# OpenVectorAI/CoFHE

Hardware: AMD Instinct MI355X
Metric: ciphertext-ops/sec + HBM GB/s (% roofline), 128x128 matadd (higher is better)
Workload: dtype u32; 1 GPU; ciphertext_matadd 128x128 per GPU (C2), security 128, k 128, |Delta| = 2088 bits, valid ciphertexts of random plaintexts; elements_per_gpu=16384, parallelism=row-shard x1, collective=none

## Files before the change

__graft_entry__.py:

```python
import json
import os
import subprocess
import sys

ROOT = os.path.dirname(os.path.abspath(__file__))
CSRC = os.path.join(ROOT, "cofhe_amd", "csrc")
LIB = os.path.join(ROOT, "cofhe_amd", "libcofhe_hip.so")
HIP_SOURCES = ["cofhe_hip.hip", "abi.hip", "kernels.hpp", "wire.hip", "shard.hip", "wide.hip", "ctx.hpp", "lane.hpp", "mp.hpp", "qf.hpp",
               "form_io.hpp", "layout.hpp", "wide.hpp", "qfw.hpp", "comb.hip", "comb.hpp", "affine.hip", "affine.hpp", "wg_ctx.hpp",
               "matmul_left.hip", "plain_mm.hpp", "conv.hip", "conv.hpp", "pow_dot.hip", "pow_dot.hpp", "poly_shift.hpp",
               "divide.hip", "plain_div.hpp", "lut.hip", "lut.hpp", "wire.hpp"]
HIP_OBJECTS = [("part0", "cofhe_hip.hip", ["-DCOFHE_PART=0"]), ("part1", "cofhe_hip.hip", ["-DCOFHE_PART=1"]),
               ("part2", "cofhe_hip.hip", ["-DCOFHE_PART=2"]), ("abi", "abi.hip", []), ("wire", "wire.hip", []), ("shard", "shard.hip", []),
               ("wide", "wide.hip", []), ("comb", "comb.hip", []), ("affine", "affine.hip", []),
               ("matmul_left", "matmul_left.hip", []), ("conv", "conv.hip", []), ("pow_dot", "pow_dot.hip", []),
               ("divide", "divide.hip", []), ("lut", "lut.hip", [])]


def _stale(target, deps):
    if not os.path.exists(target):
        return True
    t = os.path.getmtime(target)
    return any(os.path.getmtime(d) > t for d in deps)


def build_library(src_dir, obj_dir, lib, extra_flags=()) -> None:
    hipcc = os.environ.get("HIPCC", "/opt/rocm/bin/hipcc")
    flags = ["--offload-arch=gfx950", "-O2", "-std=c++17", "-fPIC", "-Wno-unused-value"] + list(extra_flags)
    os.makedirs(obj_dir, exist_ok=True)
    jobs = []
    for name, src, extra in HIP_OBJECTS:
        obj = os.path.join(obj_dir, name + ".o")
        jobs.append((obj, subprocess.Popen([hipcc] + flags + extra + ["-c", os.path.join(src_dir, src), "-o", obj], cwd=ROOT)))
    for obj, pr in jobs:
        if pr.wait() != 0:
            raise subprocess.CalledProcessError(pr.returncode, "hipcc -c -> " + obj)
    subprocess.check_call([hipcc, "--offload-arch=gfx950", "-shared", "-fPIC", "-o", lib] + [o for o, _ in jobs] + ["-ldl"], cwd=ROOT)


def build() -> None:
    deps = [os.path.join(CSRC, f) for f in HIP_SOURCES] + [os.path.join(ROOT, "include", "cofhe_hip.h")]
    if _stale(LIB, deps):
        build_library(CSRC, os.path.join(CSRC, "obj"), LIB)
    odir = os.path.join(ROOT, "oracle")
    if _stale(os.path.join(odir, "libcofhe_oracle.so"),
              [os.path.join(odir, "cofhe_oracle.hpp"), os.path.join(odir, "cofhe_oracle_c.cpp")]):
        subprocess.check_call(["make", "-C", odir])
    hdir = os.path.join(ROOT, "cofhe_amd", "host")
    exe = os.path.join(hdir, "local_bench")
    if _stale(exe, [os.path.join(hdir, f) for f in ("local_bench.cpp", "hip_cryptosystem.hpp", "smpc_local.hpp", "tensor.hpp")] + [LIB]):
        subprocess.check_call(["g++", "-std=c++17", "-O2", "-I/opt/conda/include", "-o", exe,
                               os.path.join(hdir, "local_bench.cpp"), "-L" + os.path.join(ROOT, "cofhe_amd"),
                               "-lcofhe_hip", "-l:libgmp.so.10", "-Wl,-rpath,$ORIGIN/.."], cwd=hdir)
    gdir = os.path.join(ROOT, "tests", "gpu_kernels")
    gso = os.path.join(gdir, "liblehmer_gpu.so")
    if _stale(gso, [os.path.join(gdir, "lehmer_gpu.hip"), os.path.join(CSRC, "mp.hpp"), os.path.join(CSRC, "lane.hpp")]):
        subprocess.check_call([os.environ.get("HIPCC", "/opt/rocm/bin/hipcc"), "--offload-arch=gfx950", "-O2", "-std=c++17", "-fPIC", "-shared",
                               "-Wno-unused-value", "-o", gso, os.path.join(gdir, "lehmer_gpu.hip")], cwd=ROOT)
    psrc = os.path.join(gdir, "prims_gpu.hip")
    pso = os.path.join(gdir, "libprims_gpu.so")
    pdeps = ["lane.hpp", "mp.hpp", "qf.hpp", "layout.hpp", "form_io.hpp", "wide.hpp", "qfw.hpp", "wg_ctx.hpp"]
    if os.path.exists(psrc) and _stale(pso, [psrc] + [os.path.join(CSRC, f) for f in pdeps]):
        subprocess.check_call([os.environ.get("HIPCC", "/opt/rocm/bin/hipcc"), "--offload-arch=gfx950", "-O2", "-std=c++17", "-fPIC", "-shared",
                               "-Wno-unused-value", "-o", pso, psrc], cwd=ROOT)
    lsrc = os.path.join(gdir, "lowmul_gpu.hip")
    lso = os.path.join(gdir, "liblowmul_gpu.so")
    if os.path.exists(lsrc) and _stale(lso, [lsrc] + [os.path.join(CSRC, f) for f in ("lane.hpp", "mp.hpp", "qf.hpp")]):
        subprocess.check_call([os.environ.get("HIPCC", "/opt/rocm/bin/hipcc"), "--offload-arch=gfx950", "-O2", "-std=c++17", "-fPIC", "-shared",
                               "-Wno-unused-value", "-o", lso, lsrc], cwd=ROOT)
    osrc = os.path.join(gdir, "onep_gpu.hip")
    oso = os.path.join(gdir, "libonep_gpu.so")
    if os.path.exists(osrc) and _stale(oso, [osrc] + [os.path.join(CSRC, f) for f in ("lane.hpp", "mp.hpp", "qf.hpp")]):
        subprocess.check_call([os.environ.get("HIPCC", "/opt/rocm/bin/hipcc"), "--offload-arch=gfx950", "-O2", "-std=c++17", "-fPIC", "-shared",
                               "-Wno-unused-value", "-o", oso, osrc], cwd=ROOT)
    sys.path.insert(0, ROOT)
    import cofhe_amd
    cofhe_amd.load_library()


def smoke() -> None:
    sys.path.insert(0, ROOT)
    sys.path.insert(0, os.path.join(ROOT, "tests"))
    from cofhe_amd import Engine
    import oracle_lib as O

    def hx(s):
        return -int(s[1:], 16) if s.startswith("-") else int(s, 16)

    g = os.path.join(ROOT, "tests", "golden")
    prm = json.load(open(os.path.join(g, "params_s128_k128.json")))
    vec = json.load(open(os.path.join(g, "vectors_s128_k128.json")))
    d = hx(prm["delta"])
    eng = Engine(d, device=0)
    v = vec["add_valid"]
    t1, t2 = bytes.fromhex(v["ct1"]), bytes.fromhex(v["ct2"])
    out = eng.add_ciphertext_tensors(t1, t2)
    assert out == bytes.fromhex(v["out"]), "HIP add != golden"
    assert out == O.add(d, t1, t2), "HIP add != oracle"
    v = vec["scal_2d"]
    out = eng.scal_ciphertext_tensors(bytes.fromhex(v["s"]), bytes.fromhex(v["cts"]), bytes.fromhex(v["zero"]))
    assert out == bytes.fromhex(v["out"]), "HIP scal matmul != golden"
    print("smoke ok: add_ciphertext_tensors and scal_ciphertext_tensors match golden vectors and oracle")


if __name__ == "__main__":
    build()
    if len(sys.argv) > 1 and sys.argv[1] == "smoke":
        smoke()
```

cofhe_amd/csrc/lane.hpp:

```cpp
#pragma once
#include <stdint.h>

#if defined(COFHE_HOSTSIM)
#include <atomic>
#include <cmath>
#include <cstdio>
#include <cstdlib>
#include <thread>
#define CF_DEV inline
#define CF_DEV_COLD inline
#define CF_UNROLL _Pragma("GCC unroll 16")
#define CF_NOUNROLL
#else
#include <hip/hip_runtime.h>
#define CF_DEV __device__ __forceinline__
#ifdef COFHE_COLD_CALLS
#define CF_DEV_COLD __device__ __attribute__((noinline, cold))
#else
#define CF_DEV_COLD __device__ __forceinline__
#endif
#define CF_UNROLL _Pragma("unroll")
#define CF_NOUNROLL _Pragma("nounroll")
#endif

// ... 45 lines not shown
                }
            }
        }
    }
};

struct GroupShared {
    alignas(64) uint32_t xchg[G];
    alignas(64) uint32_t own_scratch[SCRATCH_WORDS];
    uint32_t *scratch = own_scratch;
    SpinBarrier bar;
};

struct WgShared {
    SpinBarrier bar;
    SpinBarrier wave_bar;
    uint32_t vote[64];
    int wave_threads = 0;
};

struct Ctx {
    int gl;
    GroupShared *gs;
    int sense = 0;
    WgShared *wg = nullptr;
    int wg_sense = 0, wave_sense = 0;
    int tid = 0;
    uint32_t *wg_mail = nullptr, *wg_scr0 = nullptr;
    int gi = 0, wave = 0, rank = -1;
    uint32_t *scratch() const { return gs->scratch; }
};

CF_DEV void group_sync(Ctx &c) { c.gs->bar.wait(c.sense); }

CF_DEV uint32_t shfl(Ctx &c, uint32_t v, int src) {
    c.gs->xchg[c.gl] = v;
    c.gs->bar.wait(c.sense);
    uint32_t r = c.gs->xchg[src & (G - 1)];
    c.gs->bar.wait(c.sense);
    return r;
}
CF_DEV uint32_t shfl_up1(Ctx &c, uint32_t v, uint32_t fill) {
    uint32_t r = shfl(c, v, (c.gl + G - 1) & (G - 1));
    return c.gl == 0 ? fill : r;
}
CF_DEV uint32_t shfl_down1(Ctx &c, uint32_t v, uint32_t fill) {
    uint32_t r = shfl(c, v, (c.gl + 1) & (G - 1));
    return c.gl == G - 1 ? fill : r;
}
CF_DEV uint32_t shfl_xor1(Ctx &c, uint32_t v) { return shfl(c, v, c.gl ^ 1); }
CF_DEV uint32_t shfl_xor2(Ctx &c, uint32_t v) { return shfl(c, v, c.gl ^ 2); }
CF_DEV uint32_t shfl_mirror(Ctx &c, uint32_t v) { return shfl(c, v, (G - 1) - c.gl); }
CF_DEV uint32_t shfl_down4(Ctx &c, uint32_t v) { return shfl(c, v, c.gl + G / 2); }
CF_DEV uint32_t bcast_first(Ctx &c, uint32_t v) { return shfl(c, v, 0); }
CF_DEV uint32_t bcast_last(Ctx &c, uint32_t v) { return shfl(c, v, G - 1); }
CF_DEV uint32_t ballot8(Ctx &c, bool p) {
    uint32_t m = 0;
    c.gs->xchg[c.gl] = p ? 1u : 0u;
    c.gs->bar.wait(c.sense);
    for (int i = 0; i < G; i++) m |= c.gs->xchg[i] << i;
    c.gs->bar.wait(c.sense);
    return m;
}

#else

struct Ctx {
    int gl;
    int base4;
    uint32_t *scr;
    uint32_t *wg_mail = nullptr;
    uint32_t *wg_scr0 = nullptr;
    int gi = 0, wave = 0;
    int rank = 0;
    uint32_t *status = nullptr;
#ifdef COFHE_WG_TIMING
    unsigned long long t_wait = 0, t_apply = 0, n_rounds = 0, t_serve = 0;
#endif
    __device__ uint32_t *scratch() const { return scr; }
};
#define CF_ST_EUCLID_CAP 1u
#define CF_ST_REDUCE_CAP 2u
#define CF_ST_DIV_CAP 4u
#define CF_ST_BAD_FORM 8u
#define CF_ST_SCHEDULE_CAP 16u
#if !defined(COFHE_HOSTSIM)
#define CF_STATUS(c, bits) do { if ((c).status && (c).gl == 0) atomicOr((c).status, (bits)); } while (0)
#endif
#ifdef COFHE_WG_TIMING
#define CF_PHASE(id) do { if (threadIdx.x == 0) g_wg_phase[blockIdx.x * 16 + (id)] = wall_clock64(); } while (0)
#define CF_PHASE_VAL(id, v) do { if (threadIdx.x == 0) g_wg_phase[blockIdx.x * 16 + (id)] = (v); } while (0)
#define CF_FLAG(bits) do { if (c.gl == 0) atomicOr(&g_wg_flags[blockIdx.x], (bits)); } while (0)
#else
#define CF_PHASE(id) do { } while (0)
#define CF_PHASE_VAL(id, v) do { } while (0)
#define CF_FLAG(bits) do { } while (0)
#endif

CF_DEV void group_sync(Ctx &) {
    __builtin_amdgcn_fence(__ATOMIC_RELEASE, "wavefront");
    __builtin_amdgcn_wave_barrier();
    __builtin_amdgcn_fence(__ATOMIC_ACQUIRE, "wavefront");
}

CF_DEV uint32_t shfl(Ctx &c, uint32_t v, int src) {
    return (uint32_t)__builtin_amdgcn_ds_bpermute(c.base4 + ((src & (G - 1)) << 2), (int)v);
}
CF_DEV uint32_t shfl_up1(Ctx &c, uint32_t v, uint32_t fill) {
    uint32_t r = (uint32_t)__builtin_amdgcn_update_dpp((int)fill, (int)v, 0x111, 0xF, 0xF, false);
    return c.gl == 0 ? fill : r;
}
CF_DEV uint32_t shfl_down1(Ctx &c, uint32_t v, uint32_t fill) {
    uint32_t r = (uint32_t)__builtin_amdgcn_update_dpp((int)fill, (int)v, 0x101, 0xF, 0xF, false);
    return c.gl == G - 1 ? fill : r;
}
CF_DEV uint32_t shfl_xor1(Ctx &, uint32_t v) {
    return (uint32_t)__builtin_amdgcn_mov_dpp((int)v, 0xB1, 0xF, 0xF, true);
}
CF_DEV uint32_t shfl_xor2(Ctx &, uint32_t v) {
    return (uint32_t)__builtin_amdgcn_mov_dpp((int)v, 0x4E, 0xF, 0xF, true);
}
CF_DEV uint32_t shfl_mirror(Ctx &, uint32_t v) {
    return (uint32_t)__builtin_amdgcn_mov_dpp((int)v, 0x141, 0xF, 0xF, true);
}
CF_DEV uint32_t shfl_down4(Ctx &, uint32_t v) {
    return (uint32_t)__builtin_amdgcn_update_dpp((int)v, (int)v, 0x104, 0xF, 0xF, false);
}
CF_DEV uint32_t bcast_first(Ctx &, uint32_t v) {
    const int q = __builtin_amdgcn_mov_dpp((int)v, 0x00, 0xF, 0xF, true);
    return (uint32_t)__builtin_amdgcn_update_dpp(q, q, 0x141, 0xF, 0xA, false);
}
CF_DEV uint32_t bcast_last(Ctx &, uint32_t v) {
    const int q = __builtin_amdgcn_mov_dpp((int)v, 0xFF, 0xF, 0xF, true);
    return (uint32_t)__builtin_amdgcn_update_dpp(q, q, 0x141, 0xF, 0x5, false);
}
CF_DEV uint32_t ballot8(Ctx &c, bool p) {
    uint64_t m = __builtin_amdgcn_ballot_w64(p);
    return (uint32_t)(m >> (c.base4 >> 2)) & ((1u << G) - 1u);
}

#endif

CF_DEV uint32_t bcast(Ctx &c, uint32_t v, int src) { return shfl(c, v, src); }

CF_DEV bool any_lane(Ctx &c, bool p) {
#if defined(COFHE_HOSTSIM)
    return ballot8(c, p) != 0;
#else
    (void)c;
    return __builtin_amdgcn_ballot_w64(p) != 0;
#endif
}

CF_DEV uint32_t group_max(Ctx &c, uint32_t v) {
    uint32_t o;
    o = shfl_xor1(c, v); v = o > v ? o : v;
    o = shfl_xor2(c, v); v = o > v ? o : v;
    o = shfl_mirror(c, v); v = o > v ? o : v;
    return v;
}

CF_DEV int clz32(uint32_t x) { return x ? __builtin_clz(x) : 32; }

}
```

cofhe_amd/csrc/mp.hpp:

```cpp
#pragma once
#include "lane.hpp"

namespace cofhe {

#if defined(COFHE_HOSTSIM)
struct SimStats { long batches, batch_steps, divsteps, muls, divrems, resolves, bits_gained; };
inline SimStats g_stats;
#define CF_STAT(x) do { if (c.gl == 0) { x; } } while (0)
#else
#define CF_STAT(x) do { } while (0)
#endif

CF_DEV uint32_t opaque(uint32_t v) {
#if defined(COFHE_HOSTSIM)
    asm volatile("" : "+r"(v));
#else
    asm volatile("" : "+v"(v));
#endif
    return v;
}

template <int P>
struct Mp {
    uint32_t v[P][CH];
// ... 480 lines not shown
            const int k = first ? k0 + t : k1 + t - n0;
            const uint32_t *px = s + (first ? 0 : 2 * HL) + ((first ? c.gl : oc1) - k) * CH;
            const uint32_t *py = s + (first ? HL : 3 * HL) + k * CH;
            uint32_t xc[CH], yc[CH];
            CF_UNROLL for (int j = 0; j < CH; j++) {
                xc[j] = px[j];
                yc[j] = py[j];
            }
            chunk_mac(w, xc, yc);
            const bool last_of_first = (t + 1 == n0);
            CF_UNROLL for (int i = 0; i < W; i++) w0[i] = last_of_first ? w[i] : w0[i];
        }
        uint32_t bw = 0;
        CF_UNROLL for (int i = 0; i < W; i++) {
            const uint64_t d = (uint64_t)w[i] - w0[i] - bw;
            w1[i] = (uint32_t)d;
            bw = (uint32_t)(d >> 63);
        }
    }
    group_sync(c);
    uint32_t *s1 = s + G * (CH + 1);
    CF_UNROLL for (int i = 0; i < CH + 1; i++) s[c.gl * (CH + 1) + i] = w0[CH + i];
    CF_UNROLL for (int i = 0; i < W; i++) s1[oc1 * W + i] = w1[i];
    group_sync(c);
    Mp<2> r;
    uint32_t hi[2];
    {
        uint32_t cy = 0, cz = 0;
        CF_UNROLL for (int j = 0; j < CH; j++) {
            const uint32_t up = (c.gl >= 1) ? s[(c.gl >= 1 ? c.gl - 1 : 0) * (CH + 1) + j] : 0u;
            const uint32_t ov = (j == 0 && c.gl >= 2) ? s[(c.gl >= 2 ? c.gl - 2 : 0) * (CH + 1) + CH] : 0u;
            const uint64_t t = (uint64_t)w0[j] + up + ov + cy;
            r.v[0][j] = (uint32_t)t;
            cy = (uint32_t)(t >> 32);
            const uint32_t up1 = (c.gl >= 1) ? s1[(c.gl >= 1 ? c.gl - 1 : 0) * W + CH + j] : 0u;
            const uint32_t ov1 = (j == 0 && c.gl >= 2) ? s1[(c.gl >= 2 ? c.gl - 2 : 0) * W + 2 * CH] : 0u;
            const uint64_t u = (uint64_t)s1[c.gl * W + j] + up1 + ov1 + cz;
            r.v[1][j] = (uint32_t)u;
            cz = (uint32_t)(u >> 32);
        }
        hi[0] = cy;
        hi[1] = cz;
    }
    group_sync(c);
    (void)mp_resolve_sparse(c, r, hi);
    MpPair pp;
    CF_UNROLL for (int j = 0; j < CH; j++) {
        pp.p0.v[0][j] = r.v[0][j];
        pp.p1.v[0][j] = r.v[1][j];
    }
    return pp;
}

CF_DEV Mp<1> mp_sqr_low(Ctx &c, const Mp<1> &x) {
    static_assert(PLIMBS + G <= SCRATCH_WORDS && G * (CH + 1) <= SCRATCH_WORDS, "scratch too small");
    CF_STAT(g_stats.muls += 1);
    uint32_t *s = c.scratch();
    CF_UNROLL for (int j = 0; j < CH; j++) s[c.gl * CH + j] = x.v[0][j];
    s[PLIMBS + c.gl] = 0u;
    group_sync(c);
    const int kx = (mp_bitlen(c, x) + CH * 32 - 1) / (CH * 32);
    uint32_t w[2 * CH + 1];
    CF_UNROLL for (int i = 0; i < 2 * CH + 1; i++) w[i] = 0;
    CF_NOUNROLL for (int k = 0; k < kx; k++) {
        const uint32_t *px = s + ((c.gl - k) & (G - 1)) * CH;
        const uint32_t *py = (k <= c.gl) ? s + k * CH : s + PLIMBS;
        uint32_t xc[CH], yc[CH];
        CF_UNROLL for (int j = 0; j < CH; j++) {
            xc[j] = px[j];
            yc[j] = py[j];
        }
        chunk_mac(w, xc, yc);
    }
    group_sync(c);
    CF_UNROLL for (int i = 0; i < CH + 1; i++) s[c.gl * (CH + 1) + i] = w[CH + i];
    group_sync(c);
    Mp<1> r;
    uint32_t hi[1];
    {
        uint32_t cy = 0;
        CF_UNROLL for (int j = 0; j < CH; j++) {
            const uint32_t up = (c.gl >= 1) ? s[(c.gl >= 1 ? c.gl - 1 : 0) * (CH + 1) + j] : 0u;
            const uint32_t ov = (j == 0 && c.gl >= 2) ? s[(c.gl >= 2 ? c.gl - 2 : 0) * (CH + 1) + CH] : 0u;
            const uint64_t t = (uint64_t)w[j] + up + ov + cy;
            r.v[0][j] = (uint32_t)t;
            cy = (uint32_t)(t >> 32);
        }
        hi[0] = cy;
    }
    group_sync(c);
    (void)mp_resolve_sparse(c, r, hi);
    return r;
}

CF_DEV uint64_t div64_lower(uint64_t n, uint64_t d) {
    double q = (double)(n & ~0x7FFull) / (double)d;
    uint64_t t = (uint64_t)q;
    return t > 0 ? t - 1 : 0;
}

template <int PN, int PD>
CF_DEV uint32_t mp_quot_digit(Ctx &c, const Mp<PN> &num, int nb, const Mp<PD> &den, int db, int &sh) {
    int npos = nb > 64 ? nb - 64 : 0;
    int dpos = db > 32 ? db - 32 : 0;
    uint64_t nt = mp_bits64(c, num, npos);
    uint64_t dt = (uint64_t)mp_bits32(c, den, dpos) + (dpos > 0 ? 1u : 0u);
    int e = npos - dpos;
    uint64_t t;
    if (CF_UNLIKELY(dt == 0)) {
        CF_STATUS(c, CF_ST_DIV_CAP);
        sh = 0;
        return 1;
    }
    if (dpos == 0 && npos == 0) {
        t = nt / dt;
    } else {
        t = div64_lower(nt, dt);
    }
    if (e < 0) {
        t = (-e >= 64) ? 0 : (t >> (-e));
        e = 0;
    }
    int extra = 33 - __builtin_clzll(t | 1);
    if (extra > 0) {
        t >>= extra;
// ... 286 lines not shown
        WordDiv d = worddiv_make(mp_get_limb(c, den, 0));
        quot = num;
        uint32_t r = mp_divrem_word(c, quot, d);
        mp_set_word(c, num, r);
        return;
    }
    if constexpr (PD == 1) {
        mp_divrem_norm(c, num, den, db, quot);
        return;
    }
    if (db < 64) {
        mp_divrem_cons(c, num, den, quot);
        return;
    }
    mp_zero(quot);
    const int nb = mp_bitlen(c, num);
    if (nb < db) return;
    uint32_t *s = c.scratch();
    CF_UNROLL for (int p = 0; p < PD; p++)
        CF_UNROLL for (int j = 0; j < CH; j++) s[p * PLIMBS + c.gl * CH + j] = den.v[p][j];
    group_sync(c);
    const uint64_t d64 = mp_bits64(c, den, db - 64);
    const double rd = 1.0 / (double)d64;
    for (int jq = (nb - db) / 32; jq >= 0; jq--) {
        CF_STAT(g_stats.divsteps++);
        const int pos = db - 64 + 32 * jq;
        const uint64_t hi64 = mp_bits64(c, num, pos + 32);
        const uint32_t lo32 = mp_bits32(c, num, pos);
        double x = ((double)hi64 * 4294967296.0 + (double)lo32) * rd;
        x += x * 1.7763568394002505e-15;
        uint64_t qd = (uint64_t)x;
        if (qd > 0xFFFFFFFFull) qd = 0xFFFFFFFFull;
        if (qd != 0) {
            Mp<PN> ds;
            CF_UNROLL for (int p = 0; p < PN; p++)
                CF_UNROLL for (int j = 0; j < CH; j++) {
                    int i = p * PLIMBS + c.gl * CH + j - jq;
                    bool ok = i >= 0 && i < PD * PLIMBS;
                    ds.v[p][j] = ok ? s[ok ? i : 0] : 0u;
                }
            mp_lincomb_sub(c, num, 1u, num, (uint32_t)qd, ds);
            for (int fix = 0; fix < 4 && ballot8(c, c.gl == G - 1 && (num.v[PN - 1][CH - 1] >> 31)) != 0; fix++) {
                (void)mp_add(c, num, num, ds);
                qd--;
            }
        }
        CF_UNROLL for (int p = 0; p < PN; p++)
            CF_UNROLL for (int j = 0; j < CH; j++)
                quot.v[p][j] = (p * PLIMBS + c.gl * CH + j == jq) ? (uint32_t)qd : quot.v[p][j];
    }
    group_sync(c);
}

template <int PN, int PQ>
CF_DEV void mp_divexact(Ctx &c, const Mp<PN> &num, const Mp<1> &den, Mp<PQ> &quot, int nq) {
    static_assert((PN + PQ) * PLIMBS <= SCRATCH_WORDS, "scratch too small");
    mp_zero(quot);
    if (nq <= 0) return;
    if (nq > PQ * PLIMBS) nq = PQ * PLIMBS;
    const uint32_t d0raw = bcast_first(c, den.v[0][0]);
    if (CF_UNLIKELY(d0raw == 0)) {
        Mp<PN> rem = num, q;
        mp_divrem(c, rem, den, q);
        quot = mp_resize<PQ>(q);
        return;
    }
    const int tz = __builtin_ctz(d0raw);
    const Mp<1> D = mp_shr_small(c, den, tz);
    const Mp<PN> Nn = mp_shr_small(c, num, tz);
    const uint32_t d0 = d0raw >> tz | (tz ? bcast_first(c, den.v[0][1]) << (32 - tz) : 0u);
    uint32_t dinv = d0;
    CF_UNROLL for (int i = 0; i < 4; i++) dinv *= 2u - d0 * dinv;
    uint32_t *sn = c.scratch(), *sq = sn + PN * PLIMBS;
    CF_UNROLL for (int p = 0; p < PN; p++)
        CF_UNROLL for (int j = 0; j < CH; j++) sn[p * PLIMBS + c.gl * CH + j] = Nn.v[p][j];
    CF_UNROLL for (int p = 0; p < PQ; p++)
        CF_UNROLL for (int j = 0; j < CH; j++) sq[p * PLIMBS + c.gl * CH + j] = 0u;
    group_sync(c);
    Mp<1> S;
    CF_UNROLL for (int j = 0; j < CH; j++) S.v[0][j] = Nn.v[0][j];
    int64_t adj = 0;
    auto high = [&](int k) -> uint32_t { return (PLIMBS + k < PN * PLIMBS) ? sn[(PLIMBS + k < PN * PLIMBS) ? PLIMBS + k : 0] : 0u; };
    const uint64_t d64 = ((uint64_t)bcast_first(c, D.v[0][1]) << 32) | d0;
    uint64_t dinv64 = dinv;
    dinv64 *= 2ull - d64 * dinv64;
    int i = 0;
    for (; i + 1 < nq; i += 2) {
        CF_STAT(g_stats.divsteps += 2);
        const uint64_t s01 = ((uint64_t)bcast_first(c, S.v[0][1]) << 32) | bcast_first(c, S.v[0][0]);
        const uint64_t q = s01 * dinv64;
        const uint32_t q0 = (uint32_t)q, q1 = (uint32_t)(q >> 32);
        uint32_t r1[CH];
        const uint32_t hi1 = lincomb_plane<true>(r1, 1u, S.v[0], q0, D.v[0], c.gl == 0 ? q0 : 0u);
        const int64_t v1 = (int64_t)high(i) + adj + (int64_t)bcast_last(c, hi1) - (int64_t)q0;
        const int64_t adj1 = v1 >> 32;
        const uint32_t inc = shfl_up1(c, hi1, 0u);
        const uint32_t r0 = r1[0] + inc;
        const uint32_t bit = r0 < inc ? 1u : 0u;
        uint32_t s2[CH];
        s2[CH - 1] = shfl_down1(c, r0, (uint32_t)v1);
        CF_UNROLL for (int j = 0; j + 1 < CH; j++) s2[j] = r1[j + 1];
        Mp<1> T;
        uint32_t hi2[1];
        hi2[0] = lincomb_plane<true>(T.v[0], 1u, s2, q1, D.v[0], c.gl == 0 ? q1 : bit);
        const uint32_t cw = mp_resolve(c, T, hi2);
        const int64_t v2 = (int64_t)high(i + 1) + adj1 + (int64_t)cw - (int64_t)q1;
        adj = v2 >> 32;
        const uint32_t up = shfl_down1(c, T.v[0][0], (uint32_t)v2);
        CF_UNROLL for (int j = 0; j + 1 < CH; j++) S.v[0][j] = T.v[0][j + 1];
        S.v[0][CH - 1] = up;
        if (c.gl == 0) {
            sq[i] = q0;
            sq[i + 1] = q1;
        }
    }
    for (; i < nq; i++) {
        CF_STAT(g_stats.divsteps++);
        const uint32_t q = bcast_first(c, S.v[0][0]) * dinv;
        Mp<1> T;
        const uint32_t cw = mp_lincomb_sub_carry(c, T, 1u, S, q, D);
        const int64_t v = (int64_t)high(i) + adj + (int64_t)cw - (int64_t)q;
        adj = v >> 32;
        const uint32_t up = shfl_down1(c, T.v[0][0], (uint32_t)v);
        CF_UNROLL for (int j = 0; j + 1 < CH; j++) S.v[0][j] = T.v[0][j + 1];
        S.v[0][CH - 1] = up;
        if (c.gl == 0) sq[i] = q;
    }
    group_sync(c);
    CF_UNROLL for (int p = 0; p < PQ; p++)
        CF_UNROLL for (int j = 0; j < CH; j++) quot.v[p][j] = sq[p * PLIMBS + c.gl * CH + j];
    group_sync(c);
}

template <int P>
CF_DEV void smp_add(Ctx &c, SMp<P> &r, const SMp<P> &x, const SMp<P> &y) {
    if (x.neg == y.neg) {
        (void)mp_add(c, r.m, x.m, y.m);
        r.neg = x.neg;
    } else {
        int cm = mp_cmp(c, x.m, y.m);
        if (cm >= 0) {
            Mp<P> t;
            mp_sub(c, t, x.m, y.m);
            r.m = t;
            r.neg = cm == 0 ? 0 : x.neg;
        } else {
            Mp<P> t;
            mp_sub(c, t, y.m, x.m);
            r.m = t;
            r.neg = y.neg;
        }
    }
}
template <int P>
CF_DEV void smp_sub(Ctx &c, SMp<P> &r, const SMp<P> &x, const SMp<P> &y) {
    SMp<P> ny = y;
    ny.neg ^= 1;
    smp_add(c, r, x, ny);
}
template <int P, int Q>
CF_DEV SMp<P + Q> smp_mul(Ctx &c, const SMp<P> &x, const SMp<Q> &y) {
    SMp<P + Q> r;
    r.m = mp_mul(c, x.m, y.m);
    r.neg = x.neg ^ y.neg;
    return r;
}

CF_DEV void mp_bits64_pair(Ctx &c, const Mp<1> &x, const Mp<1> &y, int pos, uint64_t &xh, uint64_t &yh) {
    uint32_t *s = c.scratch();
    CF_UNROLL for (int j = 0; j < CH; j++) {
        s[c.gl * CH + j] = x.v[0][j];
        s[PLIMBS + c.gl * CH + j] = y.v[0][j];
    }
    s[2 * PLIMBS + c.gl] = 0u;
    group_sync(c);
    const int i0 = pos >> 5, o = pos & 31;
    const int i1 = i0 + 1 < PLIMBS ? i0 + 1 : 2 * PLIMBS, i2 = i0 + 2 < PLIMBS ? i0 + 2 : 2 * PLIMBS;
    const uint32_t x0 = s[i0], x1 = s[i1 < PLIMBS ? i1 : 2 * PLIMBS], x2 = s[i2 < PLIMBS ? i2 : 2 * PLIMBS];
    const uint32_t y0 = s[PLIMBS + i0], y1 = s[i1 < PLIMBS ? PLIMBS + i1 : 2 * PLIMBS],
                   y2 = s[i2 < PLIMBS ? PLIMBS + i2 : 2 * PLIMBS];
    group_sync(c);
    const uint64_t xl = ((uint64_t)x1 << 32) | x0, yl = ((uint64_t)y1 << 32) | y0;
    xh = o ? ((xl >> o) | ((uint64_t)x2 << (64 - o))) : xl;
    yh = o ? ((yl >> o) | ((uint64_t)y2 << (64 - o))) : yl;
// ... 408 lines not shown
```

cofhe_amd/csrc/qf.hpp:

```cpp
#pragma once
#include "mp.hpp"

namespace cofhe {

struct QForm {
    Mp<1> a;
    Mp<1> bm;
    int bneg;
    Mp<2> c;
};

template <int P>
CF_DEV void qf_reduce(Ctx &c, Mp<P> &a, SMp<P> &b, Mp<P> &cc) {
    for (int guard = 0;; guard++) {
        if (CF_UNLIKELY(guard > 4 * P * PLIMBS * 32)) {
            CF_STATUS(c, CF_ST_REDUCE_CAP);
            return;
        }
        int cm = mp_cmp(c, b.m, a);
        if (cm > 0 || (cm == 0 && b.neg)) {
            Mp<P> two_a;
            (void)mp_add(c, two_a, a, a);
            if (mp_cmp(c, b.m, two_a) < 0) {
                Mp<P> t;
// ... 64 lines not shown
}
CF_DEV bool m12_low_half_serves(int nb, uint32_t v1_limb0) {
    if (v1_limb0 == 0) return false;
    return nb + 1 + __builtin_ctz(v1_limb0) <= LOW2_BITS;
}
CF_DEV SMp<1> m12_low_quot(Ctx &c, const Mp<1> &pp, bool sub, int neg0, const Mp<1> &v1, int nb) {
    if (nb < 0) {
        SMp<1> z;
        mp_zero(z.m);
        z.neg = 0;
        return z;
    }
    const bool low = c.gl < LOW2_CHUNKS;
    const uint32_t flip = sub ? 0xFFFFFFFFu : 0u;
    Mp<1> n;
    uint32_t hi[1];
    {
        uint32_t cy = (sub && c.gl == 0) ? 1u : 0u;
        CF_UNROLL for (int j = 0; j < CH; j++) {
            const uint64_t t = (uint64_t)pp.v[0][j] + (shfl_down4(c, pp.v[0][j]) ^ flip) + cy;
            n.v[0][j] = (uint32_t)t;
            cy = (uint32_t)(t >> 32);
        }
        hi[0] = low ? cy : 0u;
    }
    CF_UNROLL for (int j = 0; j < CH; j++) n.v[0][j] = low ? n.v[0][j] : 0u;
    (void)mp_resolve(c, n, hi);
    CF_UNROLL for (int j = 0; j < CH; j++) n.v[0][j] = low ? n.v[0][j] : 0u;
    Mp<1> q;
    mp_divexact(c, n, v1, q, (nb + 32) >> 5);
    const int topl = nb >> 5;
    const uint32_t topmask = (2u << (nb & 31)) - 1u;
    uint32_t sbit = 0;
    CF_UNROLL for (int j = 0; j < CH; j++) sbit |= (c.gl * CH + j == topl) ? (q.v[0][j] >> (nb & 31)) & 1u : 0u;
    const bool neg = ballot8(c, sbit != 0) != 0;
    const uint32_t inv = neg ? 0xFFFFFFFFu : 0u;
    SMp<1> r;
    {
        uint32_t cy = (neg && c.gl == 0) ? 1u : 0u;
        CF_UNROLL for (int j = 0; j < CH; j++) {
            const int l = c.gl * CH + j;
            const uint32_t mask = l < topl ? 0xFFFFFFFFu : (l == topl ? topmask : 0u);
            const uint64_t t = (uint64_t)((q.v[0][j] ^ inv) & mask) + cy;
            r.m.v[0][j] = (uint32_t)t;
            cy = (uint32_t)(t >> 32);
        }
        hi[0] = cy;
    }
    (void)mp_resolve(c, r.m, hi);
    r.neg = neg0 ^ (neg ? 1 : 0);
    return r;
}

#ifdef COFHE_M12_FULL
constexpr bool M12_LOW_HALF = false;
#else
constexpr bool M12_LOW_HALF = true;
#endif

CF_DEV bool nucomp_m12(Ctx &c, SMp<1> &M1, SMp<2> &M2, const Mp<1> &R, const SMp<1> &C, const Mp<1> &v1,
                       const Mp<1> &v2, const SMp<1> &m, const SMp<1> &s, const Mp<2> &c2d, int lv1, int lv2, bool try_low) {
    if (M12_LOW_HALF && try_low) {
        const int bR = mp_bitlen(c, R), bC = mp_bitlen(c, C.m);
        const int nb1 = m12_bound(lv2, bR, mp_bitlen(c, m.m), bC, lv1);
        const int nb2 = m12_bound(mp_bitlen(c, s.m), bR, mp_bitlen(c, c2d), bC, lv1);
        const uint32_t v1w = bcast_first(c, v1.v[0][0]);
        const bool ok = m12_low_half_serves(nb1, v1w) && m12_low_half_serves(nb2, v1w);
        if (CF_LIKELY(!any_lane(c, !ok))) {
            const Mp<1> pa = mp_mul_low2(c, v2, R, m.m, C.m);
            M1 = m12_low_quot(c, pa, m.neg == C.neg, 0, v1, nb1);
            const Mp<1> pb = mp_mul_low2(c, s.m, R, mp_resize<1>(c2d), C.m);
            const SMp<1> q2 = m12_low_quot(c, pb, s.neg != C.neg, s.neg, v1, nb2);
            M2.m = mp_resize<2>(q2.m);
            M2.neg = q2.neg;
            return true;
        }
    }
    SMp<1> Rs{R, 0};
    SMp<1> v2s{v2, 0};
    SMp<2> t1 = smp_mul(c, v2s, Rs);
    SMp<2> t2 = smp_mul(c, m, C);
    SMp<2> n1;
    smp_sub(c, n1, t1, t2);
    M1 = sdiv_exact<1>(c, n1, v1);
    SMp<2> t3 = smp_mul(c, s, Rs);
    SMp<2> c2s{c2d, 0};
    SMp<3> t4w = smp_mul(c, c2s, C);
    SMp<2> t4{mp_resize<2>(t4w.m), t4w.neg};
    SMp<2> n2;
    smp_add(c, n2, t3, t4);
    M2 = sdiv_exact<2>(c, n2, v1);
    return false;
}

CF_DEV SMp<2> nucomp_dot(Ctx &c, const Mp<1> &R, const SMp<1> &C, const SMp<1> &M1, const SMp<2> &M2, bool m2_one_plane) {
    SMp<1> Rs{R, 0};
    SMp<2> p1 = smp_mul(c, Rs, M1);
    SMp<2> p2;
    if (M12_LOW_HALF && CF_LIKELY(m2_one_plane)) {
        const SMp<1> M2l{mp_resize<1>(M2.m), M2.neg};
        p2 = smp_mul(c, C, M2l);
    } else {
        SMp<3> p2w = smp_mul(c, C, M2);
        p2.m = mp_resize<2>(p2w.m);
        p2.neg = p2w.neg;
    }
    SMp<2> r;
    smp_add(c, r, p1, p2);
    return r;
}

#ifdef COFHE_DOT_FULL
constexpr bool DOT_ONE_PLANE = false;
#else
constexpr bool DOT_ONE_PLANE = true;
#endif
constexpr int DOT1_PRODUCT_BITS = PLIMBS * 32 - 3;
CF_DEV bool dot_one_plane_serves(int bR, int bC, int bM1, int bM2) {
    return bR <= LOW2_BITS && bC <= LOW2_BITS && bM1 <= LOW2_BITS && bM2 <= LOW2_BITS && bR + bM1 <= DOT1_PRODUCT_BITS &&
           bC + bM2 <= DOT1_PRODUCT_BITS;
}
// ... 335 lines not shown
                x2.m = x2p.m; x2.neg = x2p.neg ^ s.neg;
                SMp<1> sabs{s.m, 0};
                SMp<2> t = smp_mul(c, x2p, sabs);
                SMp<2> d1w{mp_resize<2>(d1), 0};
                SMp<2> t2;
                smp_sub(c, t2, t, d1w);
                y2 = sdiv_exact<1>(c, t2, d);
            }
        }
        if (mp_is_word(c, d1, 1)) {
            v1 = f1.a; v2 = f2.a; c2d = f2.c;
        } else {
            Mp<1> qq;
            v1 = f1.a; mp_divrem(c, v1, d1, qq); v1 = qq;
            v2 = f2.a; mp_divrem(c, v2, d1, qq); v2 = qq;
            Mp<3> cw = mp_mul(c, f2.c, d1);
            c2d = mp_resize<2>(cw);
        }
        const SMp<1> r0s{r, 1};
        SMp<2> num = smp_mul(c, y2, r0s);
        if (x2w != 0) {
            SMp<2> u, df;
            (void)mp_lincomb_add(c, u.m, x2w, f2.c, 0u, f2.c);
            u.neg = x2.neg;
            smp_sub(c, df, num, u);
            num = df;
        } else if (!mp_is_zero(c, x2.m)) {
            SMp<2> c2s{f2.c, 0};
            SMp<1> c2r{smod(c, c2s, v1), 0};
            SMp<2> w3 = smp_mul(c, x2, c2r), df;
            smp_sub(c, df, num, w3);
            num = df;
        }
        r = smod(c, num, v1);
    }

    CF_PHASE(3);
    const int lv1 = mp_bitlen(c, v1), lv2 = mp_bitlen(c, v2);
    int stop = (lv1 - lv2 + half_dbits) / 2;
    Euclid<1> pe;
    pe.x = v1; pe.y = r;
    mp_zero(pe.ux); mp_set_word(c, pe.uy, 1);
    pe.sx = -1; pe.sy = 1;
    qf_euclid<WG>(c, pe, stop);
    CF_PHASE(4);
#ifdef COFHE_WG_TIMING
    CF_PHASE_VAL(10, c.t_wait); CF_PHASE_VAL(11, c.t_apply); CF_PHASE_VAL(13, c.n_rounds); CF_PHASE_VAL(15, c.t_serve);
    c.t_wait = 0; c.t_apply = 0; c.n_rounds = 0; c.t_serve = 0;
#endif
    const SMp<1> C0{pe.ux, pe.sx < 0}, C1{pe.uy, pe.sy < 0};

    SMp<1> M1;
    SMp<2> M2;
    const bool m2_one_plane = nucomp_m12(c, M1, M2, pe.y, C1, v1, v2, m, s, c2d, lv1, lv2, true);
    SMp<2> an, bn;
    const bool ab_one_plane = nucomp_ab<ONE_PLANE>(c, an, bn, pe.y, C1, pe.x, C0, M1, M2, b1, m2_one_plane);
    SMp<2> cn;
    CF_PHASE(5);
    if (CF_LIKELY(ab_one_plane || (mp_high_planes_zero(c, an.m, 1) && mp_high_planes_zero(c, bn.m, 1)))) {
        (void)nucomp_c<ONE_PLANE>(c, cn.m, mp_resize<1>(an.m), mp_resize<1>(bn.m), dd);
        cn.neg = 0;
    } else {
        SMp<1> M1p;
        SMp<2> M2p;
        (void)nucomp_m12(c, M1p, M2p, pe.x, C0, v1, v2, m, s, c2d, lv1, lv2, false);
        cn = nucomp_dot(c, pe.x, C0, M1p, M2p, false);
    }

    CF_PHASE(6);
    if (CF_LIKELY(mp_bitlen(c, an.m) < PLIMBS * 32 - 8 && mp_bitlen(c, bn.m) < PLIMBS * 32 - 8 &&
                  mp_bitlen(c, cn.m) < PLIMBS * 32 - 8)) {
        Mp<1> a1 = mp_resize<1>(an.m), c1 = mp_resize<1>(cn.m);
        SMp<1> b1r{mp_resize<1>(bn.m), bn.neg};
        qf_reduce<1>(c, a1, b1r, c1);
        out.a = a1;
        out.bm = b1r.m;
        out.bneg = b1r.neg;
        out.c = mp_resize<2>(c1);
    } else {
        qf_reduce<2>(c, an.m, bn, cn.m);
        out.a = mp_resize<1>(an.m);
        out.bm = mp_resize<1>(bn.m);
        out.bneg = bn.neg;
        out.c = cn.m;
    }
    CF_PHASE(7);
}

CF_DEV void qf_inverse(Ctx &c, QForm &f) {
    if (mp_is_zero(c, f.bm)) return;
    if (mp_cmp(c, f.bm, f.a) == 0) return;
    if (mp_cmp(c, mp_resize<2>(f.a), f.c) == 0) return;
    f.bneg ^= 1;
}

constexpr uint32_t QF_BAD_SIGN_WORD = 1u << 0, QF_BAD_POSITIVE = 1u << 1, QF_BAD_B_LE_A = 1u << 2, QF_BAD_A_LE_C = 1u << 3,
                   QF_BAD_EDGE_SIGN = 1u << 4, QF_BAD_ZERO_SIGN = 1u << 5, QF_BAD_CARRY = 1u << 6, QF_BAD_LOW_BITS = 1u << 7,
                   QF_BAD_EQUATION = 1u << 8, QF_BAD_PRIMITIVE = 1u << 9;

CF_DEV uint32_t qf_form_faults(Ctx &c, const QForm &f, const uint32_t *absdelta) {
    uint32_t bad = 0;
    if (!(f.bneg == 0 || f.bneg == 1)) bad |= QF_BAD_SIGN_WORD;
    if (mp_is_zero(c, f.a)) bad |= QF_BAD_POSITIVE;
    if (mp_is_zero(c, f.c)) bad |= QF_BAD_POSITIVE;
    const Mp<2> aw = mp_resize<2>(f.a);
    const int ba = mp_cmp(c, f.bm, f.a), ac = mp_cmp(c, aw, f.c);
    if (ba > 0) bad |= QF_BAD_B_LE_A;
// ... 92 lines not shown
```

Before: 51.78 million ciphertext-ops/s.

## Pair the two M1/M2 exact divisions across lane halves and halve squaring work

Computes the two low-half NUCOMP quotients (M1, M2) together, one per half of the 8-lane group, through new paired resolve, shift and 2-limb-per-step exact-division routines. This replaces two sequential divisions. It also rewrites mp_sqr_low to compute each cross product once, double the sum, then add the diagonal terms. mp_divexact now skips high-word bookkeeping when the numerator is a single plane. The matadd benchmark may not exercise the NUCOMP path, and the new lane-half code depends on LOW2_CHUNKS=4 and on the DPP encodings being correct.

```diff
diff --git a/__graft_entry__.py b/__graft_entry__.py
--- a/__graft_entry__.py
+++ b/__graft_entry__.py
@@ -73,6 +73,11 @@
     if os.path.exists(osrc) and _stale(oso, [osrc] + [os.path.join(CSRC, f) for f in ("lane.hpp", "mp.hpp", "qf.hpp")]):
         subprocess.check_call([os.environ.get("HIPCC", "/opt/rocm/bin/hipcc"), "--offload-arch=gfx950", "-O2", "-std=c++17", "-fPIC", "-shared",
                                "-Wno-unused-value", "-o", oso, osrc], cwd=ROOT)
+    dsrc = os.path.join(gdir, "pairdiv_gpu.hip")
+    dso = os.path.join(gdir, "libpairdiv_gpu.so")
+    if os.path.exists(dsrc) and _stale(dso, [dsrc] + [os.path.join(CSRC, f) for f in ("lane.hpp", "mp.hpp", "qf.hpp")]):
+        subprocess.check_call([os.environ.get("HIPCC", "/opt/rocm/bin/hipcc"), "--offload-arch=gfx950", "-O2", "-std=c++17", "-fPIC", "-shared",
+                               "-Wno-unused-value", "-o", dso, dsrc], cwd=ROOT)
     sys.path.insert(0, ROOT)
     import cofhe_amd
     cofhe_amd.load_library()
diff --git a/cofhe_amd/csrc/lane.hpp b/cofhe_amd/csrc/lane.hpp
--- a/cofhe_amd/csrc/lane.hpp
+++ b/cofhe_amd/csrc/lane.hpp
@@ -121,6 +121,8 @@
 CF_DEV uint32_t shfl_xor2(Ctx &c, uint32_t v) { return shfl(c, v, c.gl ^ 2); }
 CF_DEV uint32_t shfl_mirror(Ctx &c, uint32_t v) { return shfl(c, v, (G - 1) - c.gl); }
 CF_DEV uint32_t shfl_down4(Ctx &c, uint32_t v) { return shfl(c, v, c.gl + G / 2); }
+CF_DEV uint32_t shfl_up4(Ctx &c, uint32_t v) { return shfl(c, v, c.gl + G / 2); }
+CF_DEV uint32_t bcast_half_first(Ctx &c, uint32_t v) { return shfl(c, v, c.gl & (G / 2)); }
 CF_DEV uint32_t bcast_first(Ctx &c, uint32_t v) { return shfl(c, v, 0); }
 CF_DEV uint32_t bcast_last(Ctx &c, uint32_t v) { return shfl(c, v, G - 1); }
 CF_DEV uint32_t ballot8(Ctx &c, bool p) {
@@ -195,6 +197,12 @@
 CF_DEV uint32_t shfl_down4(Ctx &, uint32_t v) {
     return (uint32_t)__builtin_amdgcn_update_dpp((int)v, (int)v, 0x104, 0xF, 0xF, false);
 }
+CF_DEV uint32_t shfl_up4(Ctx &, uint32_t v) {
+    return (uint32_t)__builtin_amdgcn_update_dpp((int)v, (int)v, 0x114, 0xF, 0xF, false);
+}
+CF_DEV uint32_t bcast_half_first(Ctx &, uint32_t v) {
+    return (uint32_t)__builtin_amdgcn_mov_dpp((int)v, 0x00, 0xF, 0xF, true);
+}
 CF_DEV uint32_t bcast_first(Ctx &, uint32_t v) {
     const int q = __builtin_amdgcn_mov_dpp((int)v, 0x00, 0xF, 0xF, true);
     return (uint32_t)__builtin_amdgcn_update_dpp(q, q, 0x141, 0xF, 0xA, false);
diff --git a/cofhe_amd/csrc/mp.hpp b/cofhe_amd/csrc/mp.hpp
--- a/cofhe_amd/csrc/mp.hpp
+++ b/cofhe_amd/csrc/mp.hpp
@@ -556,6 +556,11 @@
     return pp;
 }
 
+#ifdef COFHE_SQR_FULL
+constexpr bool SQR_EACH_PAIR_ONCE = false;
+#else
+constexpr bool SQR_EACH_PAIR_ONCE = true;
+#endif
 CF_DEV Mp<1> mp_sqr_low(Ctx &c, const Mp<1> &x) {
     static_assert(PLIMBS + G <= SCRATCH_WORDS && G * (CH + 1) <= SCRATCH_WORDS, "scratch too small");
     CF_STAT(g_stats.muls += 1);
@@ -563,18 +568,44 @@
     CF_UNROLL for (int j = 0; j < CH; j++) s[c.gl * CH + j] = x.v[0][j];
     s[PLIMBS + c.gl] = 0u;
     group_sync(c);
-    const int kx = (mp_bitlen(c, x) + CH * 32 - 1) / (CH * 32);
     uint32_t w[2 * CH + 1];
     CF_UNROLL for (int i = 0; i < 2 * CH + 1; i++) w[i] = 0;
-    CF_NOUNROLL for (int k = 0; k < kx; k++) {
-        const uint32_t *px = s + ((c.gl - k) & (G - 1)) * CH;
-        const uint32_t *py = (k <= c.gl) ? s + k * CH : s + PLIMBS;
-        uint32_t xc[CH], yc[CH];
-        CF_UNROLL for (int j = 0; j < CH; j++) {
-            xc[j] = px[j];
-            yc[j] = py[j];
-        }
-        chunk_mac(w, xc, yc);
+    if constexpr (SQR_EACH_PAIR_ONCE) {
+        const int noff = (c.gl + 1) >> 1;
+        CF_NOUNROLL for (int k = 0; k < G / 2; k++) {
+            const uint32_t *px = s + ((c.gl - k) & (G - 1)) * CH;
+            const uint32_t *py = (k < noff) ? s + k * CH : s + PLIMBS;
+            uint32_t xc[CH], yc[CH];
+            CF_UNROLL for (int j = 0; j < CH; j++) {
+                xc[j] = px[j];
+                yc[j] = py[j];
+            }
+            chunk_mac(w, xc, yc);
+        }
+        CF_UNROLL for (int i = 2 * CH; i > 0; i--) w[i] = (w[i] << 1) | (w[i - 1] >> 31);
+        w[0] <<= 1;
+        {
+            const uint32_t *px = s + (c.gl >> 1) * CH;
+            const uint32_t *py = (c.gl & 1) ? s + PLIMBS : px;
+            uint32_t xc[CH], yc[CH];
+            CF_UNROLL for (int j = 0; j < CH; j++) {
+                xc[j] = px[j];
+                yc[j] = py[j];
+            }
+            chunk_mac(w, xc, yc);
+        }
+    } else {
+        const int kx = (mp_bitlen(c, x) + CH * 32 - 1) / (CH * 32);
+        CF_NOUNROLL for (int k = 0; k < kx; k++) {
+            const uint32_t *px = s + ((c.gl - k) & (G - 1)) * CH;
+            const uint32_t *py = (k <= c.gl) ? s + k * CH : s + PLIMBS;
+            uint32_t xc[CH], yc[CH];
+            CF_UNROLL for (int j = 0; j < CH; j++) {
+                xc[j] = px[j];
+                yc[j] = py[j];
+            }
+            chunk_mac(w, xc, yc);
+        }
     }
     group_sync(c);
     CF_UNROLL for (int i = 0; i < CH + 1; i++) s[c.gl * (CH + 1) + i] = w[CH + i];
@@ -967,9 +998,15 @@
     group_sync(c);
 }
 
+#ifdef COFHE_DIVEXACT_HIGH
+constexpr bool DIVEXACT_HIGH_ALWAYS = true;
+#else
+constexpr bool DIVEXACT_HIGH_ALWAYS = false;
+#endif
 template <int PN, int PQ>
 CF_DEV void mp_divexact(Ctx &c, const Mp<PN> &num, const Mp<1> &den, Mp<PQ> &quot, int nq) {
     static_assert((PN + PQ) * PLIMBS <= SCRATCH_WORDS, "scratch too small");
+    constexpr bool HIGH = PN > 1 || DIVEXACT_HIGH_ALWAYS;
     mp_zero(quot);
     if (nq <= 0) return;
     if (nq > PQ * PLIMBS) nq = PQ * PLIMBS;
@@ -987,8 +1024,10 @@
     uint32_t dinv = d0;
     CF_UNROLL for (int i = 0; i < 4; i++) dinv *= 2u - d0 * dinv;
     uint32_t *sn = c.scratch(), *sq = sn + PN * PLIMBS;
-    CF_UNROLL for (int p = 0; p < PN; p++)
-        CF_UNROLL for (int j = 0; j < CH; j++) sn[p * PLIMBS + c.gl * CH + j] = Nn.v[p][j];
+    if constexpr (HIGH) {
+        CF_UNROLL for (int p = 0; p < PN; p++)
+            CF_UNROLL for (int j = 0; j < CH; j++) sn[p * PLIMBS + c.gl * CH + j] = Nn.v[p][j];
+    }
     CF_UNROLL for (int p = 0; p < PQ; p++)
         CF_UNROLL for (int j = 0; j < CH; j++) sq[p * PLIMBS + c.gl * CH + j] = 0u;
     group_sync(c);
@@ -1007,8 +1046,11 @@
         const uint32_t q0 = (uint32_t)q, q1 = (uint32_t)(q >> 32);
         uint32_t r1[CH];
         const uint32_t hi1 = lincomb_plane<true>(r1, 1u, S.v[0], q0, D.v[0], c.gl == 0 ? q0 : 0u);
-        const int64_t v1 = (int64_t)high(i) + adj + (int64_t)bcast_last(c, hi1) - (int64_t)q0;
-        const int64_t adj1 = v1 >> 32;
+        int64_t v1 = 0, adj1 = 0;
+        if constexpr (HIGH) {
+            v1 = (int64_t)high(i) + adj + (int64_t)bcast_last(c, hi1) - (int64_t)q0;
+            adj1 = v1 >> 32;
+        }
         const uint32_t inc = shfl_up1(c, hi1, 0u);
         const uint32_t r0 = r1[0] + inc;
         const uint32_t bit = r0 < inc ? 1u : 0u;
@@ -1019,8 +1061,11 @@
         uint32_t hi2[1];
         hi2[0] = lincomb_plane<true>(T.v[0], 1u, s2, q1, D.v[0], c.gl == 0 ? q1 : bit);
         const uint32_t cw = mp_resolve(c, T, hi2);
-        const int64_t v2 = (int64_t)high(i + 1) + adj1 + (int64_t)cw - (int64_t)q1;
-        adj = v2 >> 32;
+        int64_t v2 = 0;
+        if constexpr (HIGH) {
+            v2 = (int64_t)high(i + 1) + adj1 + (int64_t)cw - (int64_t)q1;
+            adj = v2 >> 32;
+        }
         const uint32_t up = shfl_down1(c, T.v[0][0], (uint32_t)v2);
         CF_UNROLL for (int j = 0; j + 1 < CH; j++) S.v[0][j] = T.v[0][j + 1];
         S.v[0][CH - 1] = up;
@@ -1034,8 +1079,11 @@
         const uint32_t q = bcast_first(c, S.v[0][0]) * dinv;
         Mp<1> T;
         const uint32_t cw = mp_lincomb_sub_carry(c, T, 1u, S, q, D);
-        const int64_t v = (int64_t)high(i) + adj + (int64_t)cw - (int64_t)q;
-        adj = v >> 32;
+        int64_t v = 0;
+        if constexpr (HIGH) {
+            v = (int64_t)high(i) + adj + (int64_t)cw - (int64_t)q;
+            adj = v >> 32;
+        }
         const uint32_t up = shfl_down1(c, T.v[0][0], (uint32_t)v);
         CF_UNROLL for (int j = 0; j + 1 < CH; j++) S.v[0][j] = T.v[0][j + 1];
         S.v[0][CH - 1] = up;
@@ -1045,6 +1093,118 @@
     CF_UNROLL for (int p = 0; p < PQ; p++)
         CF_UNROLL for (int j = 0; j < CH; j++) quot.v[p][j] = sq[p * PLIMBS + c.gl * CH + j];
     group_sync(c);
+}
+
+
+CF_DEV void mp_resolve_pair(Ctx &c, Mp<1> &r, uint32_t hi) {
+    CF_STAT(g_stats.resolves += 1);
+    const bool first = (c.gl & (LOW2_CHUNKS - 1)) == 0;
+    const uint32_t got = shfl_up1(c, hi, 0u);
+    const uint32_t inc = first ? 0u : got;
+    uint64_t t = (uint64_t)r.v[0][0] + inc;
+    r.v[0][0] = (uint32_t)t;
+    uint32_t cy = (uint32_t)(t >> 32);
+    uint32_t all = r.v[0][0];
+    CF_UNROLL for (int j = 1; j < CH; j++) {
+        t = (uint64_t)r.v[0][j] + cy;
+        r.v[0][j] = (uint32_t)t;
+        cy = (uint32_t)(t >> 32);
+        all &= r.v[0][j];
+    }
+    const uint32_t cut = 1u << (LOW2_CHUNKS - 1);
+    const uint32_t gm = ballot8(c, cy != 0) & ~cut;
+    const uint32_t pm = ballot8(c, all == 0xFFFFFFFFu && cy == 0) & ~cut;
+    const uint32_t y = gm << 1;
+    const uint32_t cin = y | (((pm + y) ^ pm) ^ y);
+    uint32_t mine = (cin >> c.gl) & 1u;
+    {
+        const uint32_t s0 = r.v[0][0] + mine;
+        mine = (s0 < mine) ? 1u : 0u;
+        r.v[0][0] = s0;
+    }
+    if (CF_UNLIKELY(any_lane(c, mine != 0))) {
+        CF_UNROLL for (int j = 1; j < CH; j++) {
+            const uint32_t s = r.v[0][j] + mine;
+            mine = (s < mine) ? 1u : 0u;
+            r.v[0][j] = s;
+        }
+    }
+}
+
+CF_DEV Mp<1> mp_shr_small_pair(Ctx &c, const Mp<1> &x, int n) {
+    Mp<1> y;
+    const uint32_t ls = (uint32_t)(32 - n) & 31u;
+    const uint32_t keep = n ? 0xFFFFFFFFu : 0u;
+    const uint32_t got = shfl_down1(c, x.v[0][0], 0u);
+    const uint32_t nxt = (c.gl & (LOW2_CHUNKS - 1)) == LOW2_CHUNKS - 1 ? 0u : got;
+    CF_UNROLL for (int j = 0; j < CH; j++) {
+        const uint32_t up = (j + 1 < CH) ? x.v[0][j + 1 < CH ? j + 1 : 0] : nxt;
+        y.v[0][j] = (x.v[0][j] >> n) | ((up << ls) & keep);
+    }
+    return y;
+}
+
+CF_DEV Mp<1> mp_divexact_pair(Ctx &c, const Mp<1> &num, const Mp<1> &den, int nq) {
+    constexpr int H = LOW2_CHUNKS, HL = H * CH;
+    static_assert(G == 8 && PLIMBS <= SCRATCH_WORDS, "scratch too small");
+    Mp<1> quot;
+    mp_zero(quot);
+    if (nq <= 0) return quot;
+    if (nq > HL) nq = HL;
+    const int oc = c.gl & (H - 1);
+    const bool low = c.gl < H;
+    const uint32_t d0raw = bcast_first(c, den.v[0][0]);
+    const int tz = __builtin_ctz(d0raw | 0x80000000u);
+    const Mp<1> Df = mp_shr_small(c, den, tz);
+    Mp<1> D;
+    CF_UNROLL for (int j = 0; j < CH; j++) {
+        const uint32_t upper = shfl_up4(c, Df.v[0][j]);
+        D.v[0][j] = low ? Df.v[0][j] : upper;
+    }
+    Mp<1> S = mp_shr_small_pair(c, num, tz);
+    const uint32_t d0 = bcast_first(c, D.v[0][0]);
+    uint32_t dinv = d0;
+    CF_UNROLL for (int i = 0; i < 4; i++) dinv *= 2u - d0 * dinv;
+    const uint64_t d64 = ((uint64_t)bcast_first(c, D.v[0][1]) << 32) | d0;
+    uint64_t dinv64 = dinv;
+    dinv64 *= 2ull - d64 * dinv64;
+    uint32_t *sq = c.scratch() + (low ? 0 : HL);
+    int i = 0;
+    for (; i + 1 < nq; i += 2) {
+        CF_STAT(g_stats.divsteps += 2);
+        const uint64_t s01 = ((uint64_t)bcast_half_first(c, S.v[0][1]) << 32) | bcast_half_first(c, S.v[0][0]);
+        const uint64_t q = s01 * dinv64;
+        const uint32_t q0 = (uint32_t)q, q1 = (uint32_t)(q >> 32);
+        uint32_t r1[CH];
+        const uint32_t hi1 = lincomb_plane<true>(r1, 1u, S.v[0], q0, D.v[0], oc == 0 ? q0 : 0u);
+        const uint32_t got = shfl_up1(c, hi1, 0u);
+        const uint32_t inc = oc == 0 ? 0u : got;
+        const uint32_t r0 = r1[0] + inc;
+        const uint32_t bit = r0 < inc ? 1u : 0u;
+        uint32_t s2[CH];
+        const uint32_t dn = shfl_down1(c, r0, 0u);
+        s2[CH - 1] = oc == H - 1 ? 0u : dn;
+        CF_UNROLL for (int j = 0; j + 1 < CH; j++) s2[j] = r1[j + 1];
+        Mp<1> T;
+        const uint32_t hi2 = lincomb_plane<true>(T.v[0], 1u, s2, q1, D.v[0], oc == 0 ? q1 : bit);
+        mp_resolve_pair(c, T, hi2);
+        const uint32_t dn2 = shfl_down1(c, T.v[0][0], 0u);
+        CF_UNROLL for (int j = 0; j + 1 < CH; j++) S.v[0][j] = T.v[0][j + 1];
+        S.v[0][CH - 1] = oc == H - 1 ? 0u : dn2;
+        if (oc == 0) {
+            sq[i] = q0;
+            sq[i + 1] = q1;
+        }
+    }
+    if (i < nq) {
+        CF_STAT(g_stats.divsteps++);
+        const uint32_t q = bcast_half_first(c, S.v[0][0]) * dinv;
+        if (oc == 0) sq[i] = q;
+    }
+    group_sync(c);
+    CF_UNROLL for (int j = 0; j < CH; j++) quot.v[0][j] = (oc * CH + j < nq) ? sq[oc * CH + j] : 0u;
+    group_sync(c);
+    return quot;
 }
 
 template <int P>
diff --git a/cofhe_amd/csrc/qf.hpp b/cofhe_amd/csrc/qf.hpp
--- a/cofhe_amd/csrc/qf.hpp
+++ b/cofhe_amd/csrc/qf.hpp
@@ -140,12 +140,65 @@
     return r;
 }
 
+struct M12Pair {
+    Mp<1> m;
+    int neg0, neg1;
+};
+CF_DEV M12Pair m12_low_quot_pair(Ctx &c, const Mp<1> &pa, const Mp<1> &pb, bool sub0, bool sub1, const Mp<1> &v1, int nb0, int nb1) {
+    const bool low = c.gl < LOW2_CHUNKS;
+    const bool first = (c.gl & (LOW2_CHUNKS - 1)) == 0;
+    const bool sub = low ? sub0 : sub1;
+    const int nb = low ? nb0 : nb1;
+    const uint32_t flip = sub ? 0xFFFFFFFFu : 0u;
+    Mp<1> n;
+    {
+        uint32_t cy = (sub && first) ? 1u : 0u;
+        CF_UNROLL for (int j = 0; j < CH; j++) {
+            const uint64_t t = (uint64_t)pa.v[0][j] + (pb.v[0][j] ^ flip) + cy;
+            n.v[0][j] = (uint32_t)t;
+            cy = (uint32_t)(t >> 32);
+        }
+        mp_resolve_pair(c, n, cy);
+    }
+    const int nbmax = nb0 > nb1 ? nb0 : nb1;
+    const Mp<1> q = mp_divexact_pair(c, n, v1, nbmax < 0 ? 0 : (nbmax + 32) >> 5);
+    const int topl = nb < 0 ? -1 : nb >> 5;
+    const uint32_t topmask = (2u << (nb & 31)) - 1u;
+    const int base = (c.gl & (LOW2_CHUNKS - 1)) * CH;
+    uint32_t sbit = 0;
+    CF_UNROLL for (int j = 0; j < CH; j++) sbit |= (base + j == topl) ? (q.v[0][j] >> (nb & 31)) & 1u : 0u;
+    const uint32_t sb = ballot8(c, sbit != 0);
+    M12Pair r;
+    r.neg0 = (sb & ((1u << LOW2_CHUNKS) - 1u)) != 0 ? 1 : 0;
+    r.neg1 = (sb >> LOW2_CHUNKS) != 0 ? 1 : 0;
+    const bool neg = (low ? r.neg0 : r.neg1) != 0;
+    const uint32_t inv = neg ? 0xFFFFFFFFu : 0u;
+    {
+        uint32_t cy = (neg && first) ? 1u : 0u;
+        CF_UNROLL for (int j = 0; j < CH; j++) {
+            const int l = base + j;
+            const uint32_t mask = l < topl ? 0xFFFFFFFFu : (l == topl ? topmask : 0u);
+            const uint64_t t = (uint64_t)((q.v[0][j] ^ inv) & mask) + cy;
+            r.m.v[0][j] = (uint32_t)t;
+            cy = (uint32_t)(t >> 32);
+        }
+        mp_resolve_pair(c, r.m, cy);
+    }
+    return r;
+}
+
 #ifdef COFHE_M12_FULL
 constexpr bool M12_LOW_HALF = false;
 #else
 constexpr bool M12_LOW_HALF = true;
 #endif
-
+#ifdef COFHE_M12_SINGLE_DIV
+constexpr bool M12_PAIRED_DIV = false;
+#else
+constexpr bool M12_PAIRED_DIV = true;
+#endif
+
+template <bool PAIRED = true>
 CF_DEV bool nucomp_m12(Ctx &c, SMp<1> &M1, SMp<2> &M2, const Mp<1> &R, const SMp<1> &C, const Mp<1> &v1,
                        const Mp<1> &v2, const SMp<1> &m, const SMp<1> &s, const Mp<2> &c2d, int lv1, int lv2, bool try_low) {
     if (M12_LOW_HALF && try_low) {
@@ -155,6 +208,21 @@
         const uint32_t v1w = bcast_first(c, v1.v[0][0]);
         const bool ok = m12_low_half_serves(nb1, v1w) && m12_low_half_serves(nb2, v1w);
         if (CF_LIKELY(!any_lane(c, !ok))) {
+            if constexpr (PAIRED && M12_PAIRED_DIV) {
+                const Mp<1> pr = mp_mul_low2(c, v2, R, s.m, R);
+                const Mp<1> pc = mp_mul_low2(c, m.m, C.m, mp_resize<1>(c2d), C.m);
+                const M12Pair qq = m12_low_quot_pair(c, pr, pc, m.neg == C.neg, s.neg != C.neg, v1, nb1, nb2);
+                const bool lowh = c.gl < LOW2_CHUNKS;
+                CF_UNROLL for (int j = 0; j < CH; j++) {
+                    const uint32_t down = shfl_down4(c, qq.m.v[0][j]);
+                    M1.m.v[0][j] = lowh ? qq.m.v[0][j] : 0u;
+                    M2.m.v[0][j] = lowh ? down : 0u;
+                    M2.m.v[1][j] = 0u;
+                }
+                M1.neg = qq.neg0;
+                M2.neg = s.neg ^ qq.neg1;
+                return true;
+            }
             const Mp<1> pa = mp_mul_low2(c, v2, R, m.m, C.m);
             M1 = m12_low_quot(c, pa, m.neg == C.neg, 0, v1, nb1);
             const Mp<1> pb = mp_mul_low2(c, s.m, R, mp_resize<1>(c2d), C.m);
@@ -596,7 +664,7 @@
 
     SMp<1> M1;
     SMp<2> M2;
-    const bool m2_one_plane = nucomp_m12(c, M1, M2, pe.y, C1, v1, v2, m, s, c2d, lv1, lv2, true);
+    const bool m2_one_plane = nucomp_m12<ONE_PLANE>(c, M1, M2, pe.y, C1, v1, v2, m, s, c2d, lv1, lv2, true);
     SMp<2> an, bn;
     const bool ab_one_plane = nucomp_ab<ONE_PLANE>(c, an, bn, pe.y, C1, pe.x, C0, M1, M2, b1, m2_one_plane);
     SMp<2> cn;
```

New measurement: 53.02 million ciphertext-ops/s (median of 6 runs). +2.4%, better.
